# ogulcanaydogan/llm-slo-ebpf-toolkit

Measured on AMD Instinct MI355X. Metric: fault-replay attribution throughput through the agent's BPF-ring -> GPU path (events/s, node-wide); held-out attribution macro-F1 and agent CPU overhead % reported alongside, higher is better.
Workload: dtype fp64 posteriors / fp32 features (exact-int64 time joins)

## Files before the change

### llm_slo_ebpf_toolkit_amd/ops/csrc/agent_bindings.cpp

```cpp
#include <pybind11/numpy.h>
#include <pybind11/pybind11.h>
#include <pybind11/stl.h>

#include <cstring>
#include <memory>
#include <stdexcept>

#include "engine.h"
#include "exemplars.h"
#include "onset.h"
#include "openreq.h"
#include "podrank.h"
#include "slisketch.h"

namespace py = pybind11;
using namespace mislo;

namespace {

template <class T>
py::array_t<T> copy_array(const T* p, std::vector<py::ssize_t> shape) {
  py::array_t<T> a(shape);
  size_t n = 1;
  for (auto s : shape) n *= (size_t)s;
// ... 687 lines not shown
    t().sync();
  }
  void close() {
    if (t_) {
      py::gil_scoped_release nogil;
      t_.reset();
    }
  }

 private:
  std::unique_ptr<OnsetTracker> t_;
};

py::bytes unique_id() {
  ncclUniqueId u;
  const ncclResult_t r = ncclGetUniqueId(&u);
  if (r != ncclSuccess) throw std::runtime_error(std::string("ncclGetUniqueId: ") + ncclGetErrorString(r));
  return py::bytes(reinterpret_cast<const char*>(&u), sizeof(u));
}

PYBIND11_MODULE(_mislo_agent, m) {
  m.doc() = "MI355X LLM-SLO native window engine (HIP + RCCL, no PyTorch)";
  m.def("set_tables", &set_tables_np);
  m.def("unique_id", &unique_id);
  m.def("device_count", []() {
    int n = 0;
    return hipGetDeviceCount(&n) == hipSuccess ? n : 0;
  });
  m.attr("PACKET_LEN") = kPacketLen;
  m.attr("PACKET_LAYOUT") = py::make_tuple(kPacketHist, kPacketStatus, kPacketMisc, kPacketDbg, kPacketConf,
                                           kPacketStats, kPacketCount, kPacketRing);
  m.attr("STATS_OFF") = kStatsOff;
  m.attr("STATS_LEN") = kStatsLen;
  m.attr("POSTERIOR_MODEL_BYTES") = (int64_t)sizeof(PosteriorModel);
  m.attr("APP_MODEL_BYTES") = (int64_t)sizeof(AppModel);
  m.attr("APP_EVIDENCE_BIT") = kAppBit;
  m.attr("CTX_ROWS") = kCtxRows;
  m.attr("REC_STRIDE") = kRecStride;
  m.attr("SIGREC_BYTES") = (int)sizeof(SigRec);
  m.attr("RING_STATE") =
      py::make_tuple("first_busy", "foreign", "def_ctx", "def_trace", "discarded", "events", "other_shard");
  m.attr("OPENREQ_LDS_GROUPS") = openreq::kLdsGroups;
  m.attr("OPENREQ_MAX_PROBES") = openreq::kMaxProbes;
  m.attr("OPENREQ_STATS") = (int)openreq::kStats;
  py::class_<PyOpenRequests>(m, "OpenRequests")
      .def(py::init<int, int64_t, int, int, int, double, double, double>(), py::arg("device") = 0,
           py::arg("cap") = (int64_t)1 << 20, py::arg("span_cap") = 16384, py::arg("group_cap") = 64,
           py::arg("n_buffers") = 3, py::arg("slo_ms") = 800.0, py::arg("ttl_ms") = 120000.0,
           py::arg("reorder_ms") = 2000.0)
      .def("step", &PyOpenRequests::step, py::arg("spans"), py::arg("cut_ns"), py::arg("prev_cut_ns"),
           py::arg("n_groups"))
      .def("query", &PyOpenRequests::query)
      .def("results", &PyOpenRequests::results)
      .def("step_ms", &PyOpenRequests::step_ms)
      .def("entries", &PyOpenRequests::entries)
      .def("sync", &PyOpenRequests::sync)
      .def("close", &PyOpenRequests::close);
  m.attr("SLISKETCH_K") = slisketch::kK;
  m.attr("SLISKETCH_LO_KEY") = slisketch::kLo;
  m.attr("SLISKETCH_STATS") = (int)slisketch::kStats;
  {
    py::list edges, q;
    for (int j = 0; j < slisketch::kEdges; ++j) edges.append((double)slisketch::le_edge(j));
    for (int j = 0; j < slisketch::kQuantiles; ++j) q.append(slisketch::quantile_permille(j));
    m.attr("SLISKETCH_EDGES") = py::tuple(edges);
    m.attr("SLISKETCH_PERMILLE") = py::tuple(q);
// ... 137 lines not shown
```

### llm_slo_ebpf_toolkit_amd/ops/csrc/bindings.cpp

```cpp
#include <torch/extension.h>
#include <c10/hip/HIPStream.h>
#include <c10/hip/HIPGuard.h>

#include <cmath>
#include <cstring>
#include <stdexcept>

#include "mislo_launch.h"
#include "mislo_packet_kernels.h"

namespace py = pybind11;
using namespace mislo;

namespace {

hipStream_t cur_stream() { return c10::hip::getCurrentHIPStream().stream(); }

#define HIPCHECK(x)                                                                    \
  do {                                                                                 \
    hipError_t _e = (x);                                                               \
    if (_e != hipSuccess) throw std::runtime_error(std::string("HIP error: ") +       \
                                                   hipGetErrorString(_e) + " at " #x); \
  } while (0)

// ... 347 lines not shown
  if (n) launch_rank_counts(vals.data_ptr<double>(), (int)n, (int)nx, dptr<uint32_t>(out), cur_stream());
  return out;
}

std::tuple<torch::Tensor, torch::Tensor> storm_counts_py(torch::Tensor keys, torch::Tensor ts, int64_t window_ns,
                                                         int64_t threshold) {
  check_dev(keys, torch::kInt64, "keys");
  check_dev(ts, torch::kInt64, "ts");
  const int64_t n = keys.numel();
  if (ts.numel() != n || n >= (1LL << 31)) throw std::invalid_argument("keys/ts size mismatch");
  c10::hip::HIPGuard guard(keys.device().index());
  auto counts = torch::empty({n}, keys.options().dtype(torch::kInt32));
  auto tally = torch::zeros({1}, keys.options());
  launch_storm_counts(dptr<uint64_t>(keys), ts.data_ptr<int64_t>(), (int)n, window_ns, (uint32_t)threshold,
                      dptr<uint32_t>(counts), dptr<unsigned long long>(tally), cur_stream());
  return {counts, tally};
}

PYBIND11_MODULE(TORCH_EXTENSION_NAME, m) {
  m.doc() = "MI355X (gfx950) LLM-SLO engine kernels";
  m.def("set_tables", &set_tables_py);
  m.def("boot_quantile", &boot_quantile_py, py::arg("sorted_c"), py::arg("sorted_b"), py::arg("q"),
        py::arg("iters"), py::arg("seed"));
  m.def("rank_counts", &rank_counts_py, py::arg("vals"), py::arg("nx"));
  m.def("storm_counts", &storm_counts_py, py::arg("keys"), py::arg("ts"), py::arg("window_ns"),
        py::arg("threshold"));
  m.attr("BOOT_MAX_N") = boot_max_n();
  m.attr("PACKET_LEN") = kPacketLen;
  m.attr("PACKET_LAYOUT") = py::make_tuple(kPacketHist, kPacketStatus, kPacketMisc, kPacketDbg, kPacketConf,
                                           kPacketStats, kPacketCount);
  m.attr("PARTS") = kParts;
  m.attr("POSTERIOR_MODEL_BYTES") = (int64_t)sizeof(PosteriorModel);
  m.attr("PROBE_PROF_OFF") = kProbeProfOff;
  py::class_<Engine>(m, "Engine")
      .def(py::init<int64_t, int64_t, int64_t, int64_t>(), py::arg("sig_cap"), py::arg("span_cap"),
           py::arg("group_cap"), py::arg("device") = 0)
      .def("set_join_params", &Engine::set_join_params, py::arg("window_ms") = 2000.0,
           py::arg("threshold") = 0.7, py::arg("fanout") = 3, py::arg("group_mode") = 1)
      .def("set_model_bytes", &Engine::set_model_bytes)
      .def("bind_io", &Engine::bind_io)
      .def("reset_window", &Engine::reset_window)
      .def("decode", &Engine::decode)
      .def("decode_ref", &Engine::decode_ref)
      .def("set_ctx_table", &Engine::set_ctx_table)
      .def("decode_ctx_wire", &Engine::decode_ctx_wire)
      .def("decode_wire", &Engine::decode_wire)
      .def("join", &Engine::join, py::arg("spans"), py::arg("n_groups"), py::arg("base_attrs") = py::none())
      .def("posterior", &Engine::posterior)
      .def("accumulate_stats", &Engine::accumulate_stats, py::arg("weights") = py::none())
      .def("pack", &Engine::pack)
      .def("run_window", &Engine::run_window, py::arg("events"), py::arg("spans"), py::arg("n_groups"),
           py::arg("with_labels") = true, py::arg("learn") = false, py::arg("wire") = 64)
      .def("refit_nb", &Engine::refit_nb, py::arg("stats_acc"), py::arg("p0"), py::arg("alpha") = 2.0,
           py::arg("prior_pseudo") = 1.0, py::arg("n_dom") = 10, py::arg("add") = py::none(), py::arg("cap_dom") = -1)
      .def("run_window_pre", &Engine::run_window_pre, py::arg("events"), py::arg("spans"), py::arg("n_groups"),
           py::arg("wire") = 64)
      .def("run_window_post", &Engine::run_window_post, py::arg("n_groups"), py::arg("with_labels") = true,
           py::arg("learn") = false)
      .def_property_readonly("sig_cap", &Engine::sig_cap)
      .def_property_readonly("span_cap", &Engine::span_cap)
      .def_property_readonly("group_cap", &Engine::group_cap)
      .def_property_readonly("packet_len", &Engine::packet_len)
#define RO(name) .def_readonly(#name, &Engine::name)
      RO(counts) RO(g_rec) RO(g_status) RO(g_part) RO(g_part_base) RO(g_items) RO(s_rec) RO(s_part)
      RO(s_part_base) RO(s_items) RO(probe_work)
      RO(top3) RO(cnt) RO(attrs) RO(conf) RO(kernel_ms) RO(gsum) RO(gcnt) RO(feat) RO(labels) RO(post)
// ... 5 lines not shown
```

### llm_slo_ebpf_toolkit_amd/ops/csrc/join.hip

```cpp
#include <cstdlib>

#include "mislo_common.h"
#include "mislo_launch.h"

namespace mislo {

constexpr int kSigBits = 27;
constexpr int kChunk = 256;


constexpr int kScanCols = 32, kScanRG = 32;
__global__ __launch_bounds__(kScanCols * kScanRG) void k_part_scan(const uint32_t* __restrict__ part_blk, int nblk,
                                                                  uint32_t* __restrict__ part_off,
                                                                  uint32_t* __restrict__ part_tot) {
  __shared__ uint32_t s_sum[kScanRG][kScanCols];
  const int cl = threadIdx.x % kScanCols, r = threadIdx.x / kScanCols;
  const int c = blockIdx.x * kScanCols + cl;
  const int per = (nblk + kScanRG - 1) / kScanRG;
  const int b0 = min(nblk, r * per), b1 = min(nblk, b0 + per);
  constexpr size_t W = (size_t)kKeyTypes * kParts;
  uint32_t sum = 0;
  for (int b = b0; b < b1; ++b) sum += part_blk[(size_t)b * W + c];
  s_sum[r][cl] = sum;
  __syncthreads();
// ... 160 lines not shown
  uint32_t slot;
};
__device__ __forceinline__ SigHot load_hot(const SigRec* p) {
  const uint4* v = reinterpret_cast<const uint4*>(p);
  const uint4 a = v[0], b = v[1], c = v[2];
  SigHot h;
  h.ts = (int64_t)(((uint64_t)a.y << 32) | a.x);
  h.tr = ((uint64_t)a.w << 32) | a.z;
  h.cn = ((uint64_t)b.y << 32) | b.x;
  h.pod = b.z;
  h.pid = b.w;
  h.sn = c.x;
  h.val = __uint_as_float(c.y);
  h.slot = c.z;
  return h;
}

struct alignas(16) SpanKT {
  uint64_t h;
  int64_t t;
};
struct alignas(16) SpanTC {
  uint64_t tr;
  uint64_t cn;
};
struct alignas(16) SpanPP {
  uint32_t pod, pid, sn, grp;
};

constexpr int kLdsGroups = 64;
constexpr int kProbeGrid = 512;
constexpr int kSigPerItem = 6144;

__device__ __forceinline__ uint32_t probe_item_class(int k, uint32_t n_sig, uint32_t n_span) {
  constexpr uint32_t kPerSig[kKeyTypes] = {90, 40, 85, 60};
  const uint32_t cost = 24000u + 64u * min(n_span, 256u) + n_sig * kPerSig[k];
  return min(cost >> 13, 63u);
}

__device__ __forceinline__ void probe_work_body(const uint32_t* __restrict__ span_base, const SignalCols& gc,
                                                const JoinParams& jp, int sig_per_item, uint32_t* __restrict__ work,
                                                unsigned long long* s, unsigned long long* s2, uint32_t* s_cls) {
  const int p = threadIdx.x;
  if (p < 64) s_cls[p] = 0u;
  const uint32_t cur = cur_slot(gc);
  const GenMeta* gm = gc.gen;
  const int64_t s_lo = gm ? ts_of_image(gm->span_lo) : INT64_MIN, s_hi = gm ? ts_of_image(gm->span_hi) : INT64_MAX;
  uint32_t ns[kKeyTypes], ng[kKeyTypes][kMaxGens], n[kKeyTypes][kMaxGens], nk[kKeyTypes];
  uint32_t b_lo[kKeyTypes][kMaxGens], b_hi[kKeyTypes][kMaxGens];
#pragma unroll
  for (int a = 0; a < kMaxGens; ++a) {
    const uint32_t* b = gc.base + (size_t)(a < gc.gens ? age_slot(gc, cur, a) : 0u) * kBaseLen;
#pragma unroll
    for (int k = 0; k < kKeyTypes; ++k) {
      b_lo[k][a] = a < gc.gens ? b[k * kParts + p] : 0u;
      b_hi[k][a] = a < gc.gens ? b[k * kParts + p + 1] : 0u;
    }
  }
#pragma unroll
  for (int k = 0; k < kKeyTypes; ++k) {
    const int c = k * kParts + p;
    ns[k] = span_base[c + 1] - span_base[c];
    nk[k] = 0;
    const int64_t w = jp.win_ns[k];
#pragma unroll
    for (int a = 0; a < kMaxGens; ++a) {
      ng[k][a] = 0;
      n[k][a] = 0;
      if (a >= gc.gens || ns[k] == 0) continue;
      const uint32_t slot = age_slot(gc, cur, a);
      if (gm) {
        if ((uint32_t)a >= gm->filled || gm->tlo[slot] > gm->thi[slot]) continue;
        const int64_t lo = max(ts_of_image(gm->tlo[slot]), gm->cut[a]), hi = ts_of_image(gm->thi[slot]);
        if (lo > hi || hi < s_lo - w || lo > s_hi + w) continue;
      }
      ng[k][a] = b_hi[k][a] - b_lo[k][a];
      n[k][a] = ng[k][a] == 0 ? 0u : min((ng[k][a] + sig_per_item - 1) / (uint32_t)sig_per_item, (uint32_t)kProbeMaxSplit);
      nk[k] += n[k][a];
    }
  }
  const unsigned long long mine = (unsigned long long)nk[0] | ((unsigned long long)nk[1] << 32);
  const unsigned long long mine2 = (unsigned long long)nk[2] | ((unsigned long long)nk[3] << 32);
  s[p] = mine;
  s2[p] = mine2;
  __syncthreads();
  for (int off = 1; off < kParts; off <<= 1) {
    const unsigned long long x = p >= off ? s[p - off] : 0ull, x2 = p >= off ? s2[p - off] : 0ull;
    __syncthreads();
    s[p] += x;
    s2[p] += x2;
    __syncthreads();
  }
  const unsigned long long tot = s[kParts - 1], tot2 = s2[kParts - 1], excl = s[p] - mine;
  const uint32_t t[kKeyTypes] = {(uint32_t)tot, (uint32_t)(tot >> 32), (uint32_t)tot2, (uint32_t)(tot2 >> 32)};
  uint32_t* items1 = work + 4;
  uint32_t* items2 = work + 4 + kProbePhaseItems;
  auto code = [&](int k, int a, uint32_t j) {
    return ((uint32_t)k << 30) | ((uint32_t)a << 28) | ((uint32_t)p << 16) | (j << 8) | n[k][a];
  };
  {
    uint32_t pos = (uint32_t)excl;
    const uint32_t sole = nk[0] == 1 ? 1u << 26 : 0u;
#pragma unroll
    for (int a = 0; a < kMaxGens; ++a)
      for (uint32_t j = 0; j < n[0][a]; ++j) items1[pos++] = code(0, a, j) | sole;
  }
  auto slice = [&](int k, int a, uint32_t j) {
    const uint32_t per = (ng[k][a] + n[k][a] - 1) / n[k][a];
    const uint32_t lo = j * per;
    return lo >= ng[k][a] ? 0u : min(ng[k][a], lo + per) - lo;
  };
#pragma unroll
  for (int k = 1; k < kKeyTypes; ++k)
#pragma unroll
    for (int a = 0; a < kMaxGens; ++a)
      for (uint32_t j = 0; j < n[k][a]; ++j) atomicAdd(&s_cls[63u - probe_item_class(k, slice(k, a, j), ns[k])], 1u);
  __syncthreads();
  if (p == 0) {
    uint32_t run = 0;
    for (int q = 0; q < 64; ++q) {
      const uint32_t v = s_cls[q];
      s_cls[q] = run;
      run += v;
    }
  }
  __syncthreads();
#pragma unroll
  for (int k = 1; k < kKeyTypes; ++k)
#pragma unroll
    for (int a = 0; a < kMaxGens; ++a)
      for (uint32_t j = 0; j < n[k][a]; ++j) {
        const uint32_t pos = atomicAdd(&s_cls[63u - probe_item_class(k, slice(k, a, j), ns[k])], 1u);
        items2[pos] = code(k, a, j);
      }
  if (p == 0) {
    work[0] = t[0];
    work[1] = t[1] + t[2] + t[3];
    work[2] = 0u;
    work[3] = 0u;
  }
}

__global__ __launch_bounds__(kParts) void k_probe_work(const uint32_t* __restrict__ span_base, SignalCols gc,
                                                       JoinParams jp, int sig_per_item, uint32_t* __restrict__ work) {
  __shared__ unsigned long long s[kParts], s2[kParts];
  __shared__ uint32_t s_cls[64];
  probe_work_body(span_base, gc, jp, sig_per_item, work, s, s2, s_cls);
}

template <int NT>
__global__ __launch_bounds__(NT) void k_scatter_sig_work(SignalCols gc, const int* __restrict__ n_ptr, int cap,
                                                         const uint32_t* __restrict__ part_off, int nblk_a,
                                                         const uint32_t* __restrict__ span_base, JoinParams jp,
                                                         int sig_per_item, uint32_t* __restrict__ work) {
  static_assert(NT == kParts, "the work-list block runs one thread per partition");
  static_assert(2 * kParts * 8 + 64 * 4 >= kKeyTypes * kParts * 4, "one LDS buffer serves both");
  __shared__ unsigned long long s_buf[2 * kParts + 32];
  if (blockIdx.x == 0) {
    probe_work_body(span_base, gc, jp, sig_per_item, work, s_buf, s_buf + kParts,
                    reinterpret_cast<uint32_t*>(s_buf + 2 * kParts));
    return;
  }
  scatter_sig_body<NT>(gc, n_ptr, cap, part_off, nblk_a, (int)blockIdx.x - 1, (int)gridDim.x - 1,
                       reinterpret_cast<uint32_t*>(s_buf));
}

template <int NT>
// ... 150 lines not shown
  __shared__ uint32_t s_i[kChunk];
  __shared__ unsigned long long s_top[kChunk * 3];
  __shared__ unsigned long long s_seed3[kChunk];
  __shared__ int s_diff[kChunk + 1];
  __shared__ int s_aux[kChunk];
  __shared__ uint16_t s_rid[kChunk];
  __shared__ uint32_t s_runok[kChunk];
  __shared__ uint16_t s_needy[kChunk];
  __shared__ int s_wsum[NT / 64];
  __shared__ int s_nneedy;
  __shared__ uint32_t s_item;
  constexpr int kLg = LG ? kLdsGroups * kSlots : 1;
  __shared__ unsigned long long s_gsum[kLg];
  __shared__ uint32_t s_gcnt[kLg];

  {
    const size_t stripe = (size_t)(blockIdx.x & (kGroupStripes - 1)) * (size_t)n_groups * kSlots;
    gsum += stripe;
    gcnt += stripe;
  }
  const bool grp_lds = LG && n_groups <= kLdsGroups;
  const bool any_groups = jp.group_mode == 1 && n_groups > 0;
  if (grp_lds && any_groups) {
    for (int i = threadIdx.x; i < kLdsGroups * kSlots; i += NT) {
      s_gsum[i] = 0ull;
      s_gcnt[i] = 0u;
    }
  }
  const bool cand1 = jp.conf[1] >= jp.threshold, cand2 = jp.conf[2] >= jp.threshold;
  unsigned long long n_cand = 0, n_low = 0, n_overlap = 0;
  const uint32_t n_work = work[phase];
  const uint32_t* items = work + 4 + (phase ? kProbePhaseItems : 0);
  const uint32_t cur = cur_slot(gc);

  for (;;) {
    __syncthreads();
    if (threadIdx.x == 0) s_item = atomicAdd(&work[2 + phase], 1u);
    __syncthreads();
    const uint32_t it = s_item;
    if (it >= n_work) break;
#ifdef MISLO_PROBE_PROFILE
    unsigned long long pt = clock64(), p_stage = 0, p_sig = 0, p_flush = 0;
#endif
    const uint32_t code = items[it];
    const int k = (int)(code >> 30);
    const int age = (int)((code >> 28) & 3u);
    const int part = (int)((code >> 16) & 0x3FF);
    const uint32_t si = (code >> 8) & 0xFF, nsplit = code & 0xFF;
    const int c = k * kParts + part;
    const uint32_t sp0 = span_base[c], sp1 = span_base[c + 1];
    const uint32_t gslot = age_slot(gc, cur, age);
    const uint32_t* sig_base = gc.base + (size_t)gslot * kBaseLen;
    const uint32_t* sig_items = gc.items + (size_t)gslot * kKeyTypes * (size_t)gc.stride;
    const KeyTs* sig_keys = gc.keys + (size_t)gslot * kKeyTypes * (size_t)gc.stride;
    const SigRec* grec = gc.rec + (size_t)gslot * (size_t)gc.stride;
    const int64_t cut = gc.gen ? gc.gen->cut[age] : INT64_MIN;
    const uint32_t n_loc = gc.gen ? gc.gen->n_local[gslot] : 0xFFFFFFFFu;
    const uint32_t cls_loc = (uint32_t)age * (uint32_t)gc.stride;
    const uint32_t cls_rem = (uint32_t)(2 * gc.gens - 1 - age) * (uint32_t)gc.stride;
    const uint32_t gb0 = sig_base[c], gb1 = sig_base[c + 1];
    const uint32_t per = (gb1 - gb0 + nsplit - 1) / nsplit;
    const uint32_t sg0 = gb0 + si * per;
    const uint32_t sg1 = min(gb1, sg0 + per);

    const int64_t w = jp.win_ns[k];
    const bool cand_tier = jp.conf[k] >= jp.threshold;
    const bool count_only = (k == 3) && !cand_tier;
    const bool track_overlap = (k < 3) && (jp.conf[3] < jp.threshold);
    const bool do_groups = cand_tier && any_groups;
    const bool ranged = (k == 1 || k == 2);

    auto add_group = [&](uint32_t grp, int slot, unsigned long long milli, uint32_t n) {
      if (grp >= (uint32_t)n_groups || n == 0) return;
      if (grp_lds) {
        atomicAdd(&s_gsum[grp * kSlots + slot], milli * n);
        atomicAdd(&s_gcnt[grp * kSlots + slot], n);
      } else {
        atomicAdd(gsum + (size_t)grp * kSlots + slot, milli * n);
        atomicAdd(gcnt + (size_t)grp * kSlots + slot, n);
      }
    };
    auto add_range = [&](int a, int b) {
      if (a < b) {
        atomicAdd(&s_diff[a], 1);
        atomicAdd(&s_diff[b], -1);
      }
    };

  for (uint32_t c0 = sp0; c0 < sp1; c0 += kChunk) {
    const int m = (int)min((uint32_t)kChunk, sp1 - c0);
    __syncthreads();
    const int ti = threadIdx.x;
    if (ti < m) {
      const uint4* src = reinterpret_cast<const uint4*>(pre + c0 + ti);
      const uint4 a = src[0], b = src[1], cc = src[2], d = src[3];
      const uint32_t my_s = d.x;
      s_kt[ti] = SpanKT{((uint64_t)a.y << 32) | a.x, (int64_t)(((uint64_t)a.w << 32) | a.z)};
      s_i[ti] = my_s;
// ... 2 lines not shown
        s_pp[ti] = SpanPP{cc.x, cc.y, cc.z, cc.w};
        s_top[3 * ti] = kEmpty;
        s_top[3 * ti + 1] = kEmpty;
        s_top[3 * ti + 2] = kEmpty;
        s_seed3[ti] = k > 0 ? top3[3ull * my_s + 2] : kEmpty;
        s_diff[ti] = 0;
        s_rid[ti] = (uint16_t)(d.y & 0xFFFFu);
        s_runok[d.y & 0xFFFFu] = d.y >> 16;
      }
    }
    if (threadIdx.x == 0 && !count_only) s_diff[m] = 0;
    __syncthreads();
    if (!count_only) {
      if (ranged) {
        for (int i = threadIdx.x; i < m; i += NT) {
          const unsigned long long seed = s_seed3[i];
          s_aux[i] = (cand_tier && (seed == kEmpty || (int)(seed >> 62) >= k)) ? 1 : 0;
        }
        __syncthreads();
        block_inclusive_scan<NT>(s_aux, m, s_wsum);
        for (int i = threadIdx.x; i < m; i += NT) {
          const int prev = i ? s_aux[i - 1] : 0;
          if (s_aux[i] != prev) s_needy[prev] = (uint16_t)i;
        }
        if (threadIdx.x == 0) s_nneedy = s_aux[m - 1];
        __syncthreads();
      }
    }
    const int n_needy = ranged && !count_only ? s_nneedy : 0;
#ifdef MISLO_PROBE_PROFILE
    { const unsigned long long t = clock64(); p_stage += t - pt; pt = t; }
#endif

    constexpr int kDepth = 1;
    uint32_t q = sg0 + threadIdx.x;
    KeyTs kq[kDepth];
    uint32_t iq[kDepth];
#pragma unroll
    for (int d = 0; d < kDepth; ++d) {
      const bool ok = q + (d + 1) * NT < sg1;
      kq[d] = ok ? sig_keys[q + (d + 1) * NT] : KeyTs{0ull, INT64_MIN};
      iq[d] = ok ? sig_items[q + (d + 1) * NT] : 0u;
    }
    auto stage1 = [&](const KeyTs& e, uint32_t idx, bool valid, int& lo, bool& vis, bool& hit, SigHot& r) {
      vis = valid && e.t >= cut;
      hit = false;
      lo = 0;
      if (!vis) return;
      lo = lower_ht(s_kt, 0, m, e.h, e.t - w);
      if (count_only) return;
      hit = lo < m && s_kt[lo].h == e.h && s_kt[lo].t <= e.t + w;
      if (hit) r = load_hot(grec + idx);
    };
    KeyTs e0 = q < sg1 ? sig_keys[q] : KeyTs{0ull, INT64_MIN};
    uint32_t i0 = q < sg1 ? sig_items[q] : 0u;
    int lo0;
    bool vis0, hit0;
    SigHot r0{};
    stage1(e0, i0, q < sg1, lo0, vis0, hit0, r0);
    for (; q < sg1; q += NT) {
      const KeyTs e1 = kq[0];
      const uint32_t i1 = iq[0];
#pragma unroll
      for (int d = 0; d + 1 < kDepth; ++d) {
        kq[d] = kq[d + 1];
        iq[d] = iq[d + 1];
      }
      {
        const bool ok = q + (kDepth + 1) * NT < sg1;
        kq[kDepth - 1] = ok ? sig_keys[q + (kDepth + 1) * NT] : KeyTs{0ull, INT64_MIN};
        iq[kDepth - 1] = ok ? sig_items[q + (kDepth + 1) * NT] : 0u;
      }
      int lo1;
      bool vis1, hit1;
      SigHot r1{};
      stage1(e1, i1, q + NT < sg1, lo1, vis1, hit1, r1);
      do {
      if (!vis0) break;
// ... 110 lines not shown
          }
        }
        if (count_cand) {
          atomicAdd(&s_diff[i], 1);
          atomicAdd(&s_diff[i + 1], -1);
          ++n_cand;
          if (fix_low) --n_low;
          if (do_groups || (k == 0 && any_groups)) {
            const uint32_t grp = pp.grp;
            if (grp != run_grp) {
              add_group(run_grp, g_slot, g_milli, run_n);
              run_grp = grp;
              run_n = 0;
            }
            ++run_n;
          }
        } else if (count_low) {
          ++n_low;
        }
        if (count_ovl) {
          const uint32_t p_sn = pp.sn;
          if ((p_sn >> 16) != 0 && (p_sn & 0xFFFF) != 0 && p_sn == g_sn && dt <= jp.win_ns[3]) ++n_overlap;
        }
      }
      add_group(run_grp, g_slot, g_milli, run_n);
      } while (0);
      e0 = e1;
      i0 = i1;
      lo0 = lo1;
      vis0 = vis1;
      hit0 = hit1;
      r0 = r1;
    }
    __syncthreads();
#ifdef MISLO_PROBE_PROFILE
    { const unsigned long long t = clock64(); p_sig += t - pt; pt = t; }
#endif
    if (!count_only) {
      block_inclusive_scan<NT>(s_diff, m, s_wsum);
      const bool sole = phase == 0 && ((code >> 26) & 1u);
      for (int i = threadIdx.x; i < m; i += NT) {
        const int nc = s_diff[i];
        const uint32_t s = s_i[i];
        if (sole) {
          cnt[s] = (uint32_t)nc;
#pragma unroll
          for (int j = 0; j < 3; ++j) top3[3ull * s + j] = s_top[3 * i + j];
          continue;
        }
        if (nc) atomicAdd(cnt + s, (uint32_t)nc);
#pragma unroll
        for (int j = 0; j < 3; ++j) {
          const unsigned long long key = s_top[3 * i + j];
          if (key == kEmpty) break;
          top3_insert(top3 + 3ull * s, key);
        }
      }
    }
#ifdef MISLO_PROBE_PROFILE
    __syncthreads();
    { const unsigned long long t = clock64(); p_flush += t - pt; pt = t; }
#endif
  }
#ifdef MISLO_PROBE_PROFILE
  if (threadIdx.x == 0) {
    unsigned long long* pr = reinterpret_cast<unsigned long long*>(work + kProbeProfOff) + 8 * k;
    atomicAdd(pr + 0, 1ull);
    atomicAdd(pr + 1, (unsigned long long)(sg1 - sg0));
    atomicAdd(pr + 2, (unsigned long long)((sp1 - sp0 + kChunk - 1) / kChunk));
    atomicAdd(pr + 3, p_stage);
    atomicAdd(pr + 4, p_sig);
    atomicAdd(pr + 5, p_flush);
  }
#endif
  }
  if (grp_lds && any_groups) {
    __syncthreads();
    for (int i = threadIdx.x; i < n_groups * kSlots; i += NT) {
      const uint32_t n = s_gcnt[i];
      if (n) {
        atomicAdd(gsum + i, s_gsum[i]);
        atomicAdd(gcnt + i, n);
      }
    }
  }
  for (int off = 32; off > 0; off >>= 1) {
    n_cand += __shfl_xor(n_cand, off);
    n_low += __shfl_xor(n_low, off);
    n_overlap += __shfl_xor(n_overlap, off);
  }
  if ((threadIdx.x & 63) == 0) {
    if (n_cand) atomicAdd(&dbg[0], n_cand);
    if (n_low) atomicAdd(&dbg[1], n_low);
    if (n_overlap) atomicAdd(&dbg[2], n_overlap);
  }
}


template <int NT>
__global__ __launch_bounds__(NT) void k_finalize(const int* __restrict__ ns_ptr, int span_cap,
                                                 const unsigned long long* __restrict__ top3,
// ... 67 lines not shown
    if (dropped) atomicAdd(&dbg[3], dropped);
    if (enriched) atomicAdd(&dbg[4], enriched);
  }
}

__device__ __forceinline__ float group_feature(unsigned long long sum, uint32_t c) {
  return c ? (float)(((double)sum * 1e-3) / (double)c) : __builtin_nanf("");
}

__global__ __launch_bounds__(256) void k_fold_groups(int n, unsigned long long* __restrict__ gsum,
                                                     uint32_t* __restrict__ gcnt, float* __restrict__ feat) {
  const int i = blockIdx.x * 256 + threadIdx.x;
  if (i >= n) return;
  unsigned long long s = gsum[i];
  uint32_t c = gcnt[i];
#pragma unroll
  for (int r = 1; r < kGroupStripes; ++r) {
    s += gsum[(size_t)r * n + i];
    c += gcnt[(size_t)r * n + i];
  }
  gsum[i] = s;
  gcnt[i] = c;
  feat[i] = group_feature(s, c);
}

__global__ __launch_bounds__(256) void k_group_features(int n, const unsigned long long* __restrict__ gsum,
                                                        const uint32_t* __restrict__ gcnt, float* __restrict__ feat) {
  const int i = blockIdx.x * 256 + threadIdx.x;
  if (i >= n) return;
  feat[i] = group_feature(gsum[i], gcnt[i]);
}


static int probe_item_signals() {
  static const int per_item = [] {
    const char* v = getenv("MISLO_PROBE_ITEM");
    const int x = v ? atoi(v) : kSigPerItem;
    return x >= 1 ? x : kSigPerItem;
  }();
  return per_item;
}

void launch_partition_sig(const SignalCols& gc, const int* n_dev, int cap, int nblk, const uint32_t* part_blk,
                          uint32_t* part_off, uint32_t* part_tot, hipStream_t stream, int nblk_a, hipEvent_t bases_done,
                          const uint32_t* work_span_base, const JoinParams* work_jp, uint32_t* work) {
  hipLaunchKernelGGL(k_part_scan, dim3(kKeyTypes * kParts / kScanCols), dim3(kScanCols * kScanRG), 0, stream,
                     part_blk, nblk, part_off, part_tot);
  hipLaunchKernelGGL(k_base_scan, dim3(1), dim3(kBaseNT), 0, stream, part_tot, gc.base, gc.gen);
  if (bases_done) (void)hipEventRecord(bases_done, stream);
  const int na = nblk_a > 0 && nblk_a < nblk ? nblk_a : nblk;
  if (work != nullptr && work_jp != nullptr && work_span_base != nullptr)
    hipLaunchKernelGGL((k_scatter_sig_work<1024>), dim3(nblk + 1), dim3(1024), 0, stream, gc, n_dev, cap, part_off,
                       na, work_span_base, *work_jp, probe_item_signals(), work);
  else
    hipLaunchKernelGGL((k_scatter_sig<1024>), dim3(nblk), dim3(1024), 0, stream, gc, n_dev, cap, part_off, na);
}

void launch_partition(const PartCodes* codes, const int* n_dev, int cap, int nblk, const uint32_t* part_blk,
                      uint32_t* part_off, uint32_t* part_tot, uint32_t* part_base, uint32_t* items,
                      hipStream_t stream, int nblk_a) {
  static_assert((kKeyTypes * kParts) % kScanCols == 0, "scan columns tile the partition matrix");
  hipLaunchKernelGGL(k_part_scan, dim3(kKeyTypes * kParts / kScanCols), dim3(kScanCols * kScanRG), 0, stream,
                     part_blk, nblk, part_off, part_tot);
  hipLaunchKernelGGL(k_base_scan, dim3(1), dim3(kBaseNT), 0, stream, part_tot, part_base, nullptr);
  hipLaunchKernelGGL((k_scatter<1024>), dim3(nblk), dim3(1024), 0, stream, codes, n_dev, cap, part_off, part_base,
                     items, nblk_a > 0 && nblk_a < nblk ? nblk_a : nblk);
}
// ... 61 lines not shown
```

### llm_slo_ebpf_toolkit_amd/ops/csrc/mislo_launch.h

```cpp
#pragma once

#include <hip/hip_runtime.h>
#include <stdint.h>

#include "mislo_common.h"
#include "mislo_packet.h"

namespace mislo {

struct PosteriorModel {
  double w[kSlots][kMaxDomains];
  double bias[kMaxDomains];
  double mean[kSlots];
  double nominal[kSlots];
  float thr[kSlots];
  uint32_t dom_mask[kMaxDomains];
  uint32_t table_mask;
  int32_t mode;
  int32_t n_pairs;
  double pair_rho;
  double w2[kSlots][kMaxPairs];
  double bias2[kMaxPairs];
  uint8_t pair_a[kMaxPairs];
  uint8_t pair_b[kMaxPairs];
};

constexpr int kAppBit = 16;
struct AppModel {
  double w[kMaxDomains];
  double b[kMaxDomains];
  double w2[kMaxPairs];
  double b2[kMaxPairs];
  double thr_ms;
  uint32_t dom_mask;
  int32_t on;
};

void set_tables(const Tables* host_tables);
int decode_grid(int cap);
// ... 47 lines not shown
void launch_remote_merge(const uint8_t* xrecv, size_t stride, int world, int me, SigRec* imp, uint32_t* remote_n,
                         uint32_t imp_cap, int max_rows, hipStream_t stream, unsigned long long* dropped = nullptr);
void launch_window_rows(const int* counts, const uint32_t* remote_n, int cap, int* rows, GenMeta* gen,
                        hipStream_t stream);
void launch_window_begin(const FillList& fl, GenMeta* gen, const GenMeta* gen_prev, unsigned long long* tmax, int gens,
                         int slots, long long halo_ns, uint32_t* ring_state, uint32_t* remote_n, const int* counts,
                         int cap, int* rows, hipStream_t stream);

void launch_partition(const PartCodes* codes, const int* n_dev, int cap, int nblk, const uint32_t* part_blk,
                      uint32_t* part_off, uint32_t* part_tot, uint32_t* part_base, uint32_t* items,
                      hipStream_t stream, int nblk_a = 0);
struct JoinParams;
void launch_partition_sig(const SignalCols& gc, const int* n_dev, int cap, int nblk, const uint32_t* part_blk,
                          uint32_t* part_off, uint32_t* part_tot, hipStream_t stream, int nblk_a = 0,
                          hipEvent_t bases_done = nullptr, const uint32_t* work_span_base = nullptr,
                          const JoinParams* work_jp = nullptr, uint32_t* work = nullptr);
struct alignas(64) PreSpan {
  uint64_t h;
  int64_t t;
  uint64_t tr, cn;
  uint32_t pod, pid, sn, grp;
  uint32_t idx, run;
  uint32_t pad[2];
};
static_assert(sizeof(PreSpan) == 64, "one cache line per staged span");
void launch_probe(const SpanCols& sc, const uint32_t* span_items, const uint32_t* span_base, const SignalCols& gc,
                  int span_cap, const JoinParams& jp, unsigned long long* top3, uint32_t* cnt, int n_groups,
                  unsigned long long* gsum, uint32_t* gcnt, unsigned long long* dbg, uint32_t* work,
                  PreSpan* span_pre, hipStream_t stream);
void launch_span_sort(const SpanCols& sc, const uint32_t* span_items, const uint32_t* span_base, PreSpan* span_pre,
                      hipStream_t stream);
void launch_probe_work(const uint32_t* span_base, const SignalCols& gc, const JoinParams& jp, uint32_t* work,
                       hipStream_t stream);
constexpr int kProbeMaxSplit = 64;
constexpr int kProbePhaseItems = kMaxGens * kParts * kProbeMaxSplit;
constexpr int kProbeProfOff = 4 + 4 * kProbePhaseItems;
constexpr int kProbeWorkLen = kProbeProfOff + 64;
void launch_finalize(const int* ns_dev, int span_cap, const unsigned long long* top3, const uint32_t* cnt,
                     const SignalCols& gc, const SpanCols& sc, const JoinParams& jp, const float* base_attrs,
                     float* attrs, float* conf, float* kernel_ms, int n_groups, unsigned long long* gsum, uint32_t* gcnt,
                     float* feat, unsigned long long* dbg, hipStream_t stream);

void launch_group_features(int n_groups, const unsigned long long* gsum, const uint32_t* gcnt, float* feat, hipStream_t stream);

void launch_posterior(const float* feat, const int* ng_dev, int cap, const PosteriorModel* pm, const int32_t* labels,
                      double* post, int32_t* pred, double* conf, uint32_t* evbits, uint32_t* confusion,
                      hipStream_t stream, const AppModel* app = nullptr, const uint32_t* app_cnt = nullptr);
void launch_stats(const float* feat, const int* ng_dev, int cap, const PosteriorModel* pm, const int32_t* labels,
                  const float* weights, double* out, double* count, hipStream_t stream);

void launch_posterior_stats(const float* feat, const int* ng_dev, int cap, const PosteriorModel* pm,
                            const int32_t* labels, double* post, int32_t* pred, double* conf, uint32_t* evbits,
                            uint32_t* confusion, const int32_t* stat_labels, const float* weights, double* out,
                            double* count, hipStream_t stream, const AppModel* app = nullptr,
                            const uint32_t* app_cnt = nullptr);
void launch_refit_nb(double* stats, const double* add, const double* p0, double alpha, double prior_pseudo, int n_dom,
                     PosteriorModel* pm, hipStream_t stream, double inv_temp = 1.0, double min_count = 0.0,
                     const double* floor_tab = nullptr, int cap_dom = -1, double ceil = 1.0);

int boot_max_n();
void launch_boot_quantile(const double* sorted_c, int nc, const double* sorted_b, int nb, double q, int iters,
                          uint64_t seed, double* out, hipStream_t stream);
void launch_rank_counts(const double* vals, int n_all, int nx, uint32_t* out, hipStream_t stream);

void launch_storm_counts(const uint64_t* keys, const int64_t* ts, int n, int64_t window_ns, uint32_t threshold,
                         uint32_t* counts, unsigned long long* n_storm, hipStream_t stream);

}
```

Before: 2.629 billion.

## Split probe work items across concatenated generations and clip signals to span reach

Probe work items are no longer split per (key type, generation). The signal ranges of all live generations for a partition are now concatenated and cut into balanced slices, and each item carries an age bitmask and loops over the generations it touches. The item cost class now weights only signals whose timestamps fall within the span window reach, and the probe loop skips signals outside [s_lo-w, s_hi+w]. This is meant to cut the number of tiny items, improve load balance, and avoid staging signals that cannot match, at the cost of a per-item generation loop and extra bookkeeping.

```diff
diff --git a/llm_slo_ebpf_toolkit_amd/ops/csrc/agent_bindings.cpp b/llm_slo_ebpf_toolkit_amd/ops/csrc/agent_bindings.cpp
--- a/llm_slo_ebpf_toolkit_amd/ops/csrc/agent_bindings.cpp
+++ b/llm_slo_ebpf_toolkit_amd/ops/csrc/agent_bindings.cpp
@@ -743,6 +743,8 @@
                                            kPacketStats, kPacketCount, kPacketRing);
   m.attr("STATS_OFF") = kStatsOff;
   m.attr("STATS_LEN") = kStatsLen;
+  m.attr("PROBE_PROF_OFF") = kProbeProfOff;
+  m.attr("PROBE_ITEM_SIGNALS") = probe_item_signals();
   m.attr("POSTERIOR_MODEL_BYTES") = (int64_t)sizeof(PosteriorModel);
   m.attr("APP_MODEL_BYTES") = (int64_t)sizeof(AppModel);
   m.attr("APP_EVIDENCE_BIT") = kAppBit;
diff --git a/llm_slo_ebpf_toolkit_amd/ops/csrc/bindings.cpp b/llm_slo_ebpf_toolkit_amd/ops/csrc/bindings.cpp
--- a/llm_slo_ebpf_toolkit_amd/ops/csrc/bindings.cpp
+++ b/llm_slo_ebpf_toolkit_amd/ops/csrc/bindings.cpp
@@ -403,6 +403,7 @@
   m.attr("PARTS") = kParts;
   m.attr("POSTERIOR_MODEL_BYTES") = (int64_t)sizeof(PosteriorModel);
   m.attr("PROBE_PROF_OFF") = kProbeProfOff;
+  m.attr("PROBE_ITEM_SIGNALS") = probe_item_signals();
   py::class_<Engine>(m, "Engine")
       .def(py::init<int64_t, int64_t, int64_t, int64_t>(), py::arg("sig_cap"), py::arg("span_cap"),
            py::arg("group_cap"), py::arg("device") = 0)
diff --git a/llm_slo_ebpf_toolkit_amd/ops/csrc/join.hip b/llm_slo_ebpf_toolkit_amd/ops/csrc/join.hip
--- a/llm_slo_ebpf_toolkit_amd/ops/csrc/join.hip
+++ b/llm_slo_ebpf_toolkit_amd/ops/csrc/join.hip
@@ -216,9 +216,10 @@
 constexpr int kProbeGrid = 512;
 constexpr int kSigPerItem = 6144;
 
-__device__ __forceinline__ uint32_t probe_item_class(int k, uint32_t n_sig, uint32_t n_span) {
+__device__ __forceinline__ uint32_t probe_item_class(int k, uint32_t n_reach, uint32_t n_rest, uint32_t n_span) {
   constexpr uint32_t kPerSig[kKeyTypes] = {90, 40, 85, 60};
-  const uint32_t cost = 24000u + 64u * min(n_span, 256u) + n_sig * kPerSig[k];
+  constexpr uint32_t kPerEntry = 6;
+  const uint32_t cost = 24000u + 64u * min(n_span, 256u) + n_reach * kPerSig[k] + n_rest * kPerEntry;
   return min(cost >> 13, 63u);
 }
 
@@ -230,7 +231,8 @@
   const uint32_t cur = cur_slot(gc);
   const GenMeta* gm = gc.gen;
   const int64_t s_lo = gm ? ts_of_image(gm->span_lo) : INT64_MIN, s_hi = gm ? ts_of_image(gm->span_hi) : INT64_MAX;
-  uint32_t ns[kKeyTypes], ng[kKeyTypes][kMaxGens], n[kKeyTypes][kMaxGens], nk[kKeyTypes];
+  uint32_t ns[kKeyTypes], len[kKeyTypes][kMaxGens], frac[kKeyTypes][kMaxGens], ages[kKeyTypes], tot[kKeyTypes],
+      n[kKeyTypes];
   uint32_t b_lo[kKeyTypes][kMaxGens], b_hi[kKeyTypes][kMaxGens];
 #pragma unroll
   for (int a = 0; a < kMaxGens; ++a) {
@@ -245,26 +247,31 @@
   for (int k = 0; k < kKeyTypes; ++k) {
     const int c = k * kParts + p;
     ns[k] = span_base[c + 1] - span_base[c];
-    nk[k] = 0;
+    ages[k] = 0u;
+    tot[k] = 0u;
     const int64_t w = jp.win_ns[k];
 #pragma unroll
     for (int a = 0; a < kMaxGens; ++a) {
-      ng[k][a] = 0;
-      n[k][a] = 0;
+      len[k][a] = 0u;
+      frac[k][a] = 256u;
       if (a >= gc.gens || ns[k] == 0) continue;
       const uint32_t slot = age_slot(gc, cur, a);
       if (gm) {
         if ((uint32_t)a >= gm->filled || gm->tlo[slot] > gm->thi[slot]) continue;
-        const int64_t lo = max(ts_of_image(gm->tlo[slot]), gm->cut[a]), hi = ts_of_image(gm->thi[slot]);
+        const int64_t t0 = ts_of_image(gm->tlo[slot]);
+        const int64_t lo = max(t0, gm->cut[a]), hi = ts_of_image(gm->thi[slot]);
         if (lo > hi || hi < s_lo - w || lo > s_hi + w) continue;
-      }
-      ng[k][a] = b_hi[k][a] - b_lo[k][a];
-      n[k][a] = ng[k][a] == 0 ? 0u : min((ng[k][a] + sig_per_item - 1) / (uint32_t)sig_per_item, (uint32_t)kProbeMaxSplit);
-      nk[k] += n[k][a];
-    }
-  }
-  const unsigned long long mine = (unsigned long long)nk[0] | ((unsigned long long)nk[1] << 32);
-  const unsigned long long mine2 = (unsigned long long)nk[2] | ((unsigned long long)nk[3] << 32);
+        const int64_t r0 = max(lo, s_lo - w), r1 = min(hi, s_hi + w);
+        frac[k][a] = (uint32_t)fminf(256.f, 1.f + 256.f * (float)(r1 - r0) / (float)(hi - t0 + 1));
+      }
+      len[k][a] = b_hi[k][a] - b_lo[k][a];
+      if (len[k][a]) ages[k] |= 1u << a;
+      tot[k] += len[k][a];
+    }
+    n[k] = probe_n_slices(tot[k], (uint32_t)sig_per_item);
+  }
+  const unsigned long long mine = (unsigned long long)n[0] | ((unsigned long long)n[1] << 32);
+  const unsigned long long mine2 = (unsigned long long)n[2] | ((unsigned long long)n[3] << 32);
   s[p] = mine;
   s2[p] = mine2;
   __syncthreads();
@@ -275,30 +282,31 @@
     s2[p] += x2;
     __syncthreads();
   }
-  const unsigned long long tot = s[kParts - 1], tot2 = s2[kParts - 1], excl = s[p] - mine;
-  const uint32_t t[kKeyTypes] = {(uint32_t)tot, (uint32_t)(tot >> 32), (uint32_t)tot2, (uint32_t)(tot2 >> 32)};
+  const unsigned long long sum = s[kParts - 1], sum2 = s2[kParts - 1], excl = s[p] - mine;
+  const uint32_t t[kKeyTypes] = {(uint32_t)sum, (uint32_t)(sum >> 32), (uint32_t)sum2, (uint32_t)(sum2 >> 32)};
   uint32_t* items1 = work + 4;
   uint32_t* items2 = work + 4 + kProbePhaseItems;
-  auto code = [&](int k, int a, uint32_t j) {
-    return ((uint32_t)k << 30) | ((uint32_t)a << 28) | ((uint32_t)p << 16) | (j << 8) | n[k][a];
+  auto code = [&](int k, uint32_t j) {
+    return ((uint32_t)k << 30) | (ages[k] << 26) | ((uint32_t)p << 16) | (j << 8) | n[k];
   };
   {
     uint32_t pos = (uint32_t)excl;
-    const uint32_t sole = nk[0] == 1 ? 1u << 26 : 0u;
-#pragma unroll
-    for (int a = 0; a < kMaxGens; ++a)
-      for (uint32_t j = 0; j < n[0][a]; ++j) items1[pos++] = code(0, a, j) | sole;
-  }
-  auto slice = [&](int k, int a, uint32_t j) {
-    const uint32_t per = (ng[k][a] + n[k][a] - 1) / n[k][a];
-    const uint32_t lo = j * per;
-    return lo >= ng[k][a] ? 0u : min(ng[k][a], lo + per) - lo;
+    for (uint32_t j = 0; j < n[0]; ++j) items1[pos++] = code(0, j);
+  }
+  auto cls = [&](int k, uint32_t j) {
+    const uint32_t v0 = probe_slice_begin(tot[k], n[k], j), v1 = probe_slice_begin(tot[k], n[k], j + 1);
+    uint32_t reach = 0;
+#pragma unroll
+    for (int a = 0; a < kMaxGens; ++a) {
+      uint32_t lo, hi;
+      if (probe_segment(len[k], a, v0, v1, &lo, &hi)) reach += ((hi - lo) * frac[k][a] + 255u) >> 8;
+    }
+    reach = min(reach, v1 - v0);
+    return 63u - probe_item_class(k, reach, v1 - v0 - reach, ns[k]);
   };
 #pragma unroll
   for (int k = 1; k < kKeyTypes; ++k)
-#pragma unroll
-    for (int a = 0; a < kMaxGens; ++a)
-      for (uint32_t j = 0; j < n[k][a]; ++j) atomicAdd(&s_cls[63u - probe_item_class(k, slice(k, a, j), ns[k])], 1u);
+    for (uint32_t j = 0; j < n[k]; ++j) atomicAdd(&s_cls[cls(k, j)], 1u);
   __syncthreads();
   if (p == 0) {
     uint32_t run = 0;
@@ -311,12 +319,7 @@
   __syncthreads();
 #pragma unroll
   for (int k = 1; k < kKeyTypes; ++k)
-#pragma unroll
-    for (int a = 0; a < kMaxGens; ++a)
-      for (uint32_t j = 0; j < n[k][a]; ++j) {
-        const uint32_t pos = atomicAdd(&s_cls[63u - probe_item_class(k, slice(k, a, j), ns[k])], 1u);
-        items2[pos] = code(k, a, j);
-      }
+    for (uint32_t j = 0; j < n[k]; ++j) items2[atomicAdd(&s_cls[cls(k, j)], 1u)] = code(k, j);
   if (p == 0) {
     work[0] = t[0];
     work[1] = t[1] + t[2] + t[3];
@@ -533,38 +536,53 @@
   const uint32_t n_work = work[phase];
   const uint32_t* items = work + 4 + (phase ? kProbePhaseItems : 0);
   const uint32_t cur = cur_slot(gc);
+  const int64_t s_lo = gc.gen ? ts_of_image(gc.gen->span_lo) : INT64_MIN;
+  const int64_t s_hi = gc.gen ? ts_of_image(gc.gen->span_hi) : INT64_MAX;
 
   for (;;) {
     __syncthreads();
     if (threadIdx.x == 0) s_item = atomicAdd(&work[2 + phase], 1u);
     __syncthreads();
-    const uint32_t it = s_item;
+    const uint32_t it = __builtin_amdgcn_readfirstlane(s_item);
     if (it >= n_work) break;
 #ifdef MISLO_PROBE_PROFILE
     unsigned long long pt = clock64(), p_stage = 0, p_sig = 0, p_flush = 0;
 #endif
     const uint32_t code = items[it];
     const int k = (int)(code >> 30);
-    const int age = (int)((code >> 28) & 3u);
+    const uint32_t ages = (code >> 26) & 0xFu;
     const int part = (int)((code >> 16) & 0x3FF);
     const uint32_t si = (code >> 8) & 0xFF, nsplit = code & 0xFF;
     const int c = k * kParts + part;
     const uint32_t sp0 = span_base[c], sp1 = span_base[c + 1];
-    const uint32_t gslot = age_slot(gc, cur, age);
-    const uint32_t* sig_base = gc.base + (size_t)gslot * kBaseLen;
-    const uint32_t* sig_items = gc.items + (size_t)gslot * kKeyTypes * (size_t)gc.stride;
-    const KeyTs* sig_keys = gc.keys + (size_t)gslot * kKeyTypes * (size_t)gc.stride;
-    const SigRec* grec = gc.rec + (size_t)gslot * (size_t)gc.stride;
-    const int64_t cut = gc.gen ? gc.gen->cut[age] : INT64_MIN;
-    const uint32_t n_loc = gc.gen ? gc.gen->n_local[gslot] : 0xFFFFFFFFu;
-    const uint32_t cls_loc = (uint32_t)age * (uint32_t)gc.stride;
-    const uint32_t cls_rem = (uint32_t)(2 * gc.gens - 1 - age) * (uint32_t)gc.stride;
-    const uint32_t gb0 = sig_base[c], gb1 = sig_base[c + 1];
-    const uint32_t per = (gb1 - gb0 + nsplit - 1) / nsplit;
-    const uint32_t sg0 = gb0 + si * per;
-    const uint32_t sg1 = min(gb1, sg0 + per);
+    uint32_t seg0[kMaxGens], seg1[kMaxGens], n_sig_item;
+    {
+      uint32_t gb[kMaxGens], glen[kMaxGens], total = 0;
+#pragma unroll
+      for (int a = 0; a < kMaxGens; ++a) {
+        gb[a] = glen[a] = 0u;
+        if ((ages >> a) & 1u) {
+          const uint32_t* sb = gc.base + (size_t)age_slot(gc, cur, a) * kBaseLen;
+          gb[a] = sb[c];
+          glen[a] = sb[c + 1] - gb[a];
+        }
+        total += glen[a];
+      }
+      const uint32_t v0 = probe_slice_begin(total, nsplit, si), v1 = probe_slice_begin(total, nsplit, si + 1);
+      n_sig_item = v1 - v0;
+#pragma unroll
+      for (int a = 0; a < kMaxGens; ++a) {
+        uint32_t lo = 0, hi = 0;
+        const bool in = probe_segment(glen, a, v0, v1, &lo, &hi);
+        seg0[a] = in ? gb[a] + lo : 0u;
+        seg1[a] = in ? gb[a] + hi : 0u;
+      }
+    }
+    (void)n_sig_item;
 
     const int64_t w = jp.win_ns[k];
+    const int64_t reach_lo = s_lo < INT64_MIN + w ? INT64_MIN : s_lo - w;
+    const int64_t reach_hi = s_hi > INT64_MAX - w ? INT64_MAX : s_hi + w;
     const bool cand_tier = jp.conf[k] >= jp.threshold;
     const bool count_only = (k == 3) && !cand_tier;
     const bool track_overlap = (k < 3) && (jp.conf[3] < jp.threshold);
@@ -633,6 +651,20 @@
     { const unsigned long long t = clock64(); p_stage += t - pt; pt = t; }
 #endif
 
+#pragma unroll 1
+    for (int age = 0; age < kMaxGens; ++age) {
+    const uint32_t sg0 = age == 0 ? seg0[0] : age == 1 ? seg0[1] : age == 2 ? seg0[2] : seg0[3];
+    const uint32_t sg1 = age == 0 ? seg1[0] : age == 1 ? seg1[1] : age == 2 ? seg1[2] : seg1[3];
+    if (sg0 >= sg1) continue;
+    const uint32_t gslot = age_slot(gc, cur, age);
+    const uint32_t* sig_items = gc.items + (size_t)gslot * kKeyTypes * (size_t)gc.stride;
+    const KeyTs* sig_keys = gc.keys + (size_t)gslot * kKeyTypes * (size_t)gc.stride;
+    const SigRec* grec = gc.rec + (size_t)gslot * (size_t)gc.stride;
+    const int64_t cut = gc.gen ? gc.gen->cut[age] : INT64_MIN;
+    const int64_t vis_lo = max(cut, reach_lo);
+    const uint32_t n_loc = gc.gen ? gc.gen->n_local[gslot] : 0xFFFFFFFFu;
+    const uint32_t cls_loc = (uint32_t)age * (uint32_t)gc.stride;
+    const uint32_t cls_rem = (uint32_t)(2 * gc.gens - 1 - age) * (uint32_t)gc.stride;
     constexpr int kDepth = 1;
     uint32_t q = sg0 + threadIdx.x;
     KeyTs kq[kDepth];
@@ -644,7 +676,7 @@
       iq[d] = ok ? sig_items[q + (d + 1) * NT] : 0u;
     }
     auto stage1 = [&](const KeyTs& e, uint32_t idx, bool valid, int& lo, bool& vis, bool& hit, SigHot& r) {
-      vis = valid && e.t >= cut;
+      vis = valid && e.t >= vis_lo && e.t <= reach_hi;
       hit = false;
       lo = 0;
       if (!vis) return;
@@ -821,13 +853,14 @@
       hit0 = hit1;
       r0 = r1;
     }
+    }
     __syncthreads();
 #ifdef MISLO_PROBE_PROFILE
     { const unsigned long long t = clock64(); p_sig += t - pt; pt = t; }
 #endif
     if (!count_only) {
       block_inclusive_scan<NT>(s_diff, m, s_wsum);
-      const bool sole = phase == 0 && ((code >> 26) & 1u);
+      const bool sole = phase == 0 && nsplit == 1u;
       for (int i = threadIdx.x; i < m; i += NT) {
         const int nc = s_diff[i];
         const uint32_t s = s_i[i];
@@ -855,7 +888,7 @@
   if (threadIdx.x == 0) {
     unsigned long long* pr = reinterpret_cast<unsigned long long*>(work + kProbeProfOff) + 8 * k;
     atomicAdd(pr + 0, 1ull);
-    atomicAdd(pr + 1, (unsigned long long)(sg1 - sg0));
+    atomicAdd(pr + 1, (unsigned long long)n_sig_item);
     atomicAdd(pr + 2, (unsigned long long)((sp1 - sp0 + kChunk - 1) / kChunk));
     atomicAdd(pr + 3, p_stage);
     atomicAdd(pr + 4, p_sig);
@@ -989,7 +1022,7 @@
 }
 
 
-static int probe_item_signals() {
+int probe_item_signals() {
   static const int per_item = [] {
     const char* v = getenv("MISLO_PROBE_ITEM");
     const int x = v ? atoi(v) : kSigPerItem;
diff --git a/llm_slo_ebpf_toolkit_amd/ops/csrc/mislo_launch.h b/llm_slo_ebpf_toolkit_amd/ops/csrc/mislo_launch.h
--- a/llm_slo_ebpf_toolkit_amd/ops/csrc/mislo_launch.h
+++ b/llm_slo_ebpf_toolkit_amd/ops/csrc/mislo_launch.h
@@ -5,6 +5,7 @@
 
 #include "mislo_common.h"
 #include "mislo_packet.h"
+#include "probe_items.h"
 
 namespace mislo {
 
@@ -118,10 +119,11 @@
                       hipStream_t stream);
 void launch_probe_work(const uint32_t* span_base, const SignalCols& gc, const JoinParams& jp, uint32_t* work,
                        hipStream_t stream);
-constexpr int kProbeMaxSplit = 64;
+static_assert(kProbeMaxGens == kMaxGens, "the item code's age mask has one bit per generation");
 constexpr int kProbePhaseItems = kMaxGens * kParts * kProbeMaxSplit;
 constexpr int kProbeProfOff = 4 + 4 * kProbePhaseItems;
 constexpr int kProbeWorkLen = kProbeProfOff + 64;
+int probe_item_signals();
 void launch_finalize(const int* ns_dev, int span_cap, const unsigned long long* top3, const uint32_t* cnt,
                      const SignalCols& gc, const SpanCols& sc, const JoinParams& jp, const float* base_attrs,
                      float* attrs, float* conf, float* kernel_ms, int n_groups, unsigned long long* gsum, uint32_t* gcnt,
diff --git a/llm_slo_ebpf_toolkit_amd/ops/csrc/probe_items.h b/llm_slo_ebpf_toolkit_amd/ops/csrc/probe_items.h
--- /dev/null
+++ b/llm_slo_ebpf_toolkit_amd/ops/csrc/probe_items.h
@@ -0,0 +1,42 @@
+#pragma once
+
+#include <stdint.h>
+
+#if defined(__HIPCC__) || defined(__CUDACC__)
+#define MISLO_PI_FN __host__ __device__ inline
+#else
+#define MISLO_PI_FN inline
+#endif
+
+namespace mislo {
+
+constexpr int kProbeMaxGens = 4;
+constexpr int kProbeMaxSplit = 64;
+
+MISLO_PI_FN uint32_t probe_n_slices(uint32_t total, uint32_t per_item) {
+  if (total == 0) return 0u;
+  if (per_item == 0) per_item = 1u;
+  const uint32_t n = total / per_item + (total % per_item ? 1u : 0u);
+  return n < (uint32_t)kProbeMaxSplit ? n : (uint32_t)kProbeMaxSplit;
+}
+
+MISLO_PI_FN uint32_t probe_slice_begin(uint32_t total, uint32_t n, uint32_t j) {
+  const uint32_t q = total / n, r = total % n;
+  return j * q + (j < r ? j : r);
+}
+
+MISLO_PI_FN bool probe_segment(const uint32_t len[kProbeMaxGens], int age, uint32_t v0, uint32_t v1, uint32_t* lo,
+                               uint32_t* hi) {
+  uint32_t off = 0;
+  for (int a = 0; a < age; ++a) off += len[a];
+  const uint32_t end = off + len[age];
+  const uint32_t b = v0 > off ? v0 : off, e = v1 < end ? v1 : end;
+  if (b >= e) return false;
+  *lo = b - off;
+  *hi = e - off;
+  return true;
+}
+
+}
+
+#undef MISLO_PI_FN
```

Result: slower. 2.590 billion (-1.5%).
